# huzi96/gaussian-pcloud-render

Hardware: AMD Instinct MI355X
Metric: rendered frames/sec at 1080p (fwd+bwd), THuman-800K (higher is better)
Workload: dtype f32

## Files before the change

### gaussian-pcloud-render_amd/csrc/binning.hip

```cpp
#include "common.hpp"
#include "tile_cull.hpp"

namespace gsr {

__device__ __forceinline__ uint64_t agent_load(const uint64_t* p)
{
    return __hip_atomic_load(p, __ATOMIC_RELAXED, __HIP_MEMORY_SCOPE_AGENT);
}
__device__ __forceinline__ void agent_store(uint64_t* p, uint64_t v)
{
    __hip_atomic_store(p, v, __ATOMIC_RELAXED, __HIP_MEMORY_SCOPE_AGENT);
}

#ifdef GSR_STATS
constexpr int DUP_REC = 65536;
__device__ unsigned g_dup_rec[DUP_REC][4];
#define DUP_T(var) const unsigned long long var = wall_clock64()
#define DUP_ADD(i, v) do { if (threadIdx.x == 0) { const unsigned r_ = blockIdx.y * gridDim.x + s_ticket; if (r_ < DUP_REC) g_dup_rec[r_][i] = (unsigned)(v); } } while (0)
int debug_dup_times(unsigned long long* out8, int reset)
{
    static unsigned host[DUP_REC][4];
    if (hipMemcpyFromSymbol(host, HIP_SYMBOL(g_dup_rec), sizeof(host)) != hipSuccess) return -1;
    for (int i = 0; i < 8; i++) out8[i] = 0;
    for (int r = 0; r < DUP_REC; r++) {
// ... 272 lines not shown
    return check_launch(L, "duplicate");
}

constexpr int RANGE_SAMPLE = 4096;
constexpr int RANGE_MAX_SAMPLES = 8192;

template <typename KeyT>
__device__ __forceinline__ uint32_t lower_bound_keys(const KeyT* __restrict__ keys, uint32_t n, const uint32_t* __restrict__ samples,
                                                     uint32_t ns, uint32_t t)
{
    uint32_t lo = 0, hi = n;
    if (ns != 0) {
        uint32_t a = 0, b = ns;
        while (a < b) {
            const uint32_t m = (a + b) >> 1;
            if (samples[m] < t) a = m + 1; else b = m;
        }
        if (a == 0) return 0;
        lo = (a - 1) * RANGE_SAMPLE + 1;
        hi = a < ns ? a * RANGE_SAMPLE : n;
    }
    while (lo < hi) {
        const uint32_t m = (lo + hi) >> 1;
        if ((uint32_t)keys[m] < t) lo = m + 1; else hi = m;
    }
    return lo;
}

constexpr int RANGE_TILES_PER_WG = 255;
template <typename KeyT>
__global__ __launch_bounds__(256) void k_tile_ranges(const uint64_t* __restrict__ counters, size_t g_stride, int64_t cap,
                                                     const KeyT* __restrict__ keys, size_t b_stride, uint2* __restrict__ ranges,
                                                     size_t iv_stride, int T)
{
    __shared__ uint32_t samples[RANGE_MAX_SAMPLES];
    __shared__ uint32_t bound[256];
    const uint32_t view = blockIdx.y;
    const uint64_t n64 = at_view(counters, g_stride, view)[CNT_NUM_RENDERED];
    const uint32_t n = (uint32_t)(n64 < (uint64_t)cap ? n64 : (uint64_t)cap);
    keys = at_view(keys, b_stride, view);
    ranges = at_view(ranges, iv_stride, view);
    uint32_t ns = (n + RANGE_SAMPLE - 1) / RANGE_SAMPLE;
    if (ns > RANGE_MAX_SAMPLES) ns = 0;
    for (uint32_t j = threadIdx.x; j < ns; j += 256) samples[j] = (uint32_t)keys[(size_t)j * RANGE_SAMPLE];
    __syncthreads();
    const int t = blockIdx.x * RANGE_TILES_PER_WG + threadIdx.x;
    bound[threadIdx.x] = (t < T && n != 0) ? lower_bound_keys(keys, n, samples, ns, (uint32_t)t) : n;
    __syncthreads();
    if (threadIdx.x >= RANGE_TILES_PER_WG || t >= T) return;
    const uint32_t first = bound[threadIdx.x], last = bound[threadIdx.x + 1];
    ranges[t] = first < last ? make_uint2(first, last) : make_uint2(0u, 0u);
}

int launch_tile_ranges(const Launch& L, const Batch& B, const uint32_t* sorted_keys, int T, bool key16)
{
    const dim3 grid((unsigned)div_up(T, RANGE_TILES_PER_WG), B.V);
    if (key16)
        hipLaunchKernelGGL(k_tile_ranges<uint16_t>, grid, dim3(256), 0, L.stream, B.g.counters, B.g_stride, B.b.cap,
                           (const uint16_t*)sorted_keys, B.b_stride, B.iv.ranges, B.iv_stride, T);
    else
        hipLaunchKernelGGL(k_tile_ranges<uint32_t>, grid, dim3(256), 0, L.stream, B.g.counters, B.g_stride, B.b.cap, sorted_keys,
                           B.b_stride, B.iv.ranges, B.iv_stride, T);
    return check_launch(L, "tile_ranges");
}

constexpr int ORD_BUCKETS = 128;

__device__ __forceinline__ uint32_t work_bucket(uint32_t len)
{
    if (len == 0) return ORD_BUCKETS - 1;
    const uint32_t msb = 31u - (uint32_t)__builtin_clz(len);
    const uint32_t frac = msb >= 2 ? (len >> (msb - 2)) & 3u : 0u;
    const uint32_t rank = msb * 4u + frac;
    return (ORD_BUCKETS - 2) - (rank < ORD_BUCKETS - 2 ? rank : ORD_BUCKETS - 2);
}

__device__ __forceinline__ uint32_t work_estimate(uint32_t len, float knee, float expo)
{
    if (knee <= 0.f || (float)len <= knee) return len;
    return (uint32_t)(knee * __builtin_amdgcn_exp2f(expo * __builtin_amdgcn_logf(knee / (float)len)));
}

__global__ __launch_bounds__(1024) void k_tile_order(int T, const uint2* __restrict__ ranges, uint32_t* __restrict__ tile_order,
                                                     size_t iv_stride, float knee, float expo)
{
    ranges = at_view(ranges, iv_stride, blockIdx.x);
    tile_order = at_view(tile_order, iv_stride, blockIdx.x);
    __shared__ uint32_t cnt[ORD_BUCKETS];
    __shared__ uint32_t cur[ORD_BUCKETS];
    const uint32_t lane = threadIdx.x & 63;
    const uint64_t lt_mask = (1ull << lane) - 1ull;
    if (threadIdx.x < ORD_BUCKETS) cnt[threadIdx.x] = 0;
    __syncthreads();
    const int T_pad = (T + 1023) / 1024 * 1024;
    for (int pass = 0; pass < 2; pass++) {
        for (int t = threadIdx.x; t < T_pad; t += 1024) {
            const bool ok = t < T;
            uint32_t b = 0;
            if (ok) b = work_bucket(work_estimate(ranges[t].y - ranges[t].x, knee, expo));
            const bool empty = ok && b == ORD_BUCKETS - 1;
            const uint64_t em = __ballot(empty);
            uint32_t slot = 0;
            if (pass == 0) {
                if (empty) { if ((em & lt_mask) == 0) atomicAdd(&cnt[b], (uint32_t)__popcll(em)); }
                else if (ok) atomicAdd(&cnt[b], 1u);
            } else {
                uint32_t basev = 0;
                const int leader = em ? (int)__builtin_ctzll(em) : 0;
                if (empty && (int)lane == leader) basev = atomicAdd(&cur[b], (uint32_t)__popcll(em));
                basev = __shfl(basev, leader, 64);
                if (empty) slot = basev + (uint32_t)__popcll(em & lt_mask);
                else if (ok) slot = atomicAdd(&cur[b], 1u);
                if (ok) tile_order[slot] = (uint32_t)t;
            }
        }
        __syncthreads();
        if (pass == 0) {
            if (threadIdx.x < 64) {
                const uint32_t a0 = cnt[2 * lane], a1 = cnt[2 * lane + 1];
                uint32_t inc = a0 + a1;
#pragma unroll
                for (int d = 1; d < 64; d <<= 1) {
                    const uint32_t n = __shfl_up(inc, d, 64);
                    if (lane >= (uint32_t)d) inc += n;
                }
                cur[2 * lane] = inc - a0 - a1;
                cur[2 * lane + 1] = inc - a1;
            }
            __syncthreads();
        }
    }
}

static void order_params(float& knee, float& expo)
{
    static const float k = [] { const char* e = getenv("GSR_ORDER_KNEE"); return e ? (float)atof(e) : 2048.f; }();
    static const float x = [] { const char* e = getenv("GSR_ORDER_EXP"); return e ? (float)atof(e) : 0.3f; }();
    knee = k;
    expo = x;
}

int launch_tile_order(const Launch& L, const Batch& B, int T)
{
    float knee, expo;
    order_params(knee, expo);
    hipLaunchKernelGGL(k_tile_order, dim3(B.V), dim3(1024), 0, L.stream, T, B.iv.ranges, B.iv.tile_order, B.iv_stride, knee, expo);
    return check_launch(L, "tile_order");
}

constexpr int BWD_CLEAR_BLOCKS = 64;
__global__ __launch_bounds__(1024) void k_bwd_items(int T, int chunk_shift, const uint32_t* __restrict__ need, uint32_t* __restrict__ items,
                                                    uint32_t* __restrict__ count, size_t iv_stride, const uint64_t* __restrict__ counters,
                                                    size_t g_stride, float* __restrict__ grad_rec, size_t gr_stride, size_t gr_bytes)
{
    if (blockIdx.y != 0) {
        if (at_view(counters, g_stride, blockIdx.x)[CNT_BWD_DIRTY] == 0) return;
        zero_region(reinterpret_cast<char*>(at_view(grad_rec, gr_stride, blockIdx.x)), gr_bytes,
                    (size_t)(blockIdx.y - 1) * 1024 + threadIdx.x, (size_t)BWD_CLEAR_BLOCKS * 1024);
        return;
    }
    need = at_view(need, iv_stride, blockIdx.x);
    items = at_view(items, iv_stride, blockIdx.x);
    count = at_view(count, iv_stride, blockIdx.x);
    if (threadIdx.x < 8) count[BWD_QUEUE_WORD + threadIdx.x] = 0;
    __shared__ uint32_t cnt[ORD_BUCKETS];
    __shared__ uint32_t cur[ORD_BUCKETS];
    const uint32_t lane = threadIdx.x & 63;
    if (threadIdx.x < ORD_BUCKETS) cnt[threadIdx.x] = 0;
    __syncthreads();
    const uint32_t full_bucket = work_bucket(1u << chunk_shift);
    for (int pass = 0; pass < 2; pass++) {
        for (int t = threadIdx.x; t < T; t += 1024) {
            const uint32_t n = need[t];
            if (n == 0) continue;
            uint32_t n_full = n >> chunk_shift;
            if (n_full > BWD_MAX_CHUNKS - 1) n_full = BWD_MAX_CHUNKS - 1;
            const uint32_t rest = n - (n_full << chunk_shift);
            if (pass == 0) {
                if (n_full) atomicAdd(&cnt[full_bucket], n_full);
                if (rest) atomicAdd(&cnt[work_bucket(rest)], 1u);
            } else {
                if (n_full) {
                    const uint32_t slot = atomicAdd(&cur[full_bucket], n_full);
                    for (uint32_t c = 0; c < n_full; c++) items[slot + c] = (uint32_t)t | (c << BWD_TILE_BITS);
                }
                if (rest) items[atomicAdd(&cur[work_bucket(rest)], 1u)] = (uint32_t)t | (n_full << BWD_TILE_BITS);
            }
        }
        __syncthreads();
        if (pass == 0) {
            if (threadIdx.x < 64) {
                const uint32_t a0 = cnt[2 * lane], a1 = cnt[2 * lane + 1];
                uint32_t inc = a0 + a1;
#pragma unroll
                for (int d = 1; d < 64; d <<= 1) {
                    const uint32_t n = __shfl_up(inc, d, 64);
                    if (lane >= (uint32_t)d) inc += n;
                }
                cur[2 * lane] = inc - a0 - a1;
                cur[2 * lane + 1] = inc - a1;
                if (lane == 63) count[0] = inc;
            }
            __syncthreads();
        }
    }
}

int launch_bwd_items(const Launch& L, const Batch& B, int T, int P)
{
    hipLaunchKernelGGL(k_bwd_items, dim3(B.V, 1 + BWD_CLEAR_BLOCKS), dim3(1024), 0, L.stream, T, B.chunk_shift(), B.iv.tile_need, B.iv.bwd_items,
                       B.iv.bwd_count, B.iv_stride, B.g.counters, B.g_stride, B.grad_rec, B.gr_stride, grad_rec_bytes(P));
    return check_launch(L, "bwd_items");
}

}
```

### gaussian-pcloud-render_amd/csrc/common.hpp

```cpp
#pragma once
#include <hip/hip_runtime.h>
#include <stdint.h>

#include <type_traits>

#include "../../include/gsr.h"

#if defined(__HIP_DEVICE_COMPILE__) && !defined(__gfx950__)
#error "libgsr_hip is written for gfx950 (MI355X) only: build with --offload-arch=gfx950"
#endif

namespace gsr {

constexpr int TILE_X = 16;
constexpr int TILE_Y = 16;
constexpr int TILE_PIX = TILE_X * TILE_Y;

constexpr int RS_THREADS = 256;
constexpr int RS_WAVES = RS_THREADS / 64;
#ifndef GSR_RS_ITEMS
#define GSR_RS_ITEMS 16
#endif
constexpr int RS_ITEMS = GSR_RS_ITEMS;
constexpr int RS_TILE = RS_THREADS * RS_ITEMS;
constexpr int RADIX_BITS = 8;
constexpr int RADIX = 1 << RADIX_BITS;

constexpr int RS_ITEMS_SMALL = 8;
constexpr int RS_TILE_SMALL = RS_THREADS * RS_ITEMS_SMALL;
inline int sort_hist_stride(int64_t n, int tile = RS_TILE) { return (int)(((n + tile - 1) / tile + 15) / 16 * 16); }

constexpr int DUP_THREADS = 256;
#ifndef GSR_DUP_G
#define GSR_DUP_G 4
#endif
constexpr int DUP_G = GSR_DUP_G;
constexpr int DUP_BLOCK = DUP_THREADS * DUP_G;
#ifndef GSR_DUP_COPIES
#define GSR_DUP_COPIES 8
#endif
constexpr int DUP_COPIES = GSR_DUP_COPIES;

inline size_t align_up(size_t v, size_t a) { return (v + a - 1) / a * a; }
inline int64_t div_up(int64_t a, int64_t b) { return (a + b - 1) / b; }

template <typename T>
__host__ __device__ __forceinline__ T* at_view(T* p, size_t stride_bytes, uint32_t view)
{
    using B = typename std::conditional<std::is_const<T>::value, const char, char>::type;
    return (T*)((B*)p + stride_bytes * view);
}

struct __attribute__((aligned(64))) Splat {
    float4 q0, q1, q2, q3;
};

constexpr int GRAD_REC_WORDS = 16;
inline size_t grad_rec_bytes(int P) { return ((size_t)(P > 0 ? P : 1) * GRAD_REC_WORDS * sizeof(float) + 255) / 256 * 256; }

constexpr int CNT_NUM_RENDERED = 0;
constexpr int CNT_TRAP = 1;
constexpr int CNT_STALL = 2;
constexpr int CNT_NUM_REFERENCE = 4;
constexpr int LAND_NUM_REFERENCE = 3;
constexpr int CNT_BWD_DIRTY = 3;

struct GeomView {
    Splat* splat;
    uint32_t* tiles_touched;
    uint8_t* clamped;
    uint32_t* dkey[2];
    uint32_t* dval[2];
    uint32_t* hist;
    uint32_t* totals;
    uint32_t* blk_minmax;
    uint32_t* sortctl;
    uint64_t* dup_status;
    uint64_t* counters;
    char* zero_begin;
    size_t zero_bytes;
    size_t bytes;
};

constexpr int BWD_CHUNK_SHIFT_MIN = 9;
#ifndef GSR_CHUNK_V
#define GSR_CHUNK_V 2
#endif
__host__ __device__ inline int bwd_chunk_shift(int V) { return V >= GSR_CHUNK_V ? 10 : 9; }
constexpr int BWD_MAX_CHUNKS = 32;
constexpr int BWD_QUEUE_WORD = 8;
constexpr int BWD_TILE_BITS = 27;

struct BinView {
    uint32_t* key[2];
    uint32_t* val[2];
    uint32_t* hist;
    uint32_t* totals;
    float4* ckpt;
    int64_t cap;
    size_t bytes;
};

struct ImageView {
    uint32_t* tile_need;
    uint32_t* bwd_count;
    uint2* ranges;
    float* final_T;
    uint32_t* n_contrib;
    uint32_t* tile_order;
    float* accum;
    uint32_t* bwd_items;
    char* zero_begin;
    size_t zero_bytes;
    size_t bytes;
};

template <typename T>
inline void carve(char*& cur, T*& ptr, size_t count)
{
    ptr = reinterpret_cast<T*>(cur);
    cur += align_up(count * sizeof(T), 256);
}

inline GeomView geom_view(void* base, int P)
{
    GeomView g;
    char* cur = reinterpret_cast<char*>(base);
    const size_t p = (size_t)(P > 0 ? P : 1);
    const size_t nblk = (size_t)sort_hist_stride((int64_t)p, RS_TILE_SMALL);
    carve(cur, g.splat, p);
    carve(cur, g.tiles_touched, p);
    carve(cur, g.clamped, p);
    carve(cur, g.dkey[0], p);
    carve(cur, g.dkey[1], p);
    carve(cur, g.dval[0], p);
    carve(cur, g.dval[1], p);
    carve(cur, g.hist, RADIX * nblk);
    carve(cur, g.totals, (size_t)RADIX);
    carve(cur, g.blk_minmax, 2 * nblk);
    carve(cur, g.sortctl, (size_t)4);
    g.zero_begin = cur;
// ... 222 lines not shown
```

### gaussian-pcloud-render_amd/csrc/preprocess.hip

```cpp
#include "common.hpp"
#include "splat_math.hpp"
#include "tile_cull.hpp"

namespace gsr {

template <int deg>
__device__ __forceinline__ V3 sh_to_rgb_t(V3 pos, V3 campos, const float* sh, uint32_t* clamp_mask)
{
    V3 dir = pos - campos;
    const float len = sqrtf(dot3(dir, dir));
    dir = v3(dir.x / len, dir.y / len, dir.z / len);
#define SHV(k) v3(sh[3 * (k)], sh[3 * (k) + 1], sh[3 * (k) + 2])
    V3 result = kSH_C0 * SHV(0);
    if constexpr (deg > 0) {
        const float x = dir.x, y = dir.y, z = dir.z;
        result = ((result - (kSH_C1 * y) * SHV(1)) + (kSH_C1 * z) * SHV(2)) - (kSH_C1 * x) * SHV(3);
        if constexpr (deg > 1) {
            const float xx = x * x, yy = y * y, zz = z * z;
            const float xy = x * y, yz = y * z, xz = x * z;
            result = result + (kSH_C2[0] * xy) * SHV(4);
            result = result + (kSH_C2[1] * yz) * SHV(5);
            result = result + (kSH_C2[2] * (2.0f * zz - xx - yy)) * SHV(6);
            result = result + (kSH_C2[3] * xz) * SHV(7);
            result = result + (kSH_C2[4] * (xx - yy)) * SHV(8);
            if constexpr (deg > 2) {
                result = result + (kSH_C3[0] * y * (3.0f * xx - yy)) * SHV(9);
                result = result + (kSH_C3[1] * xy * z) * SHV(10);
                result = result + (kSH_C3[2] * y * (4.0f * zz - xx - yy)) * SHV(11);
                result = result + (kSH_C3[3] * z * (2.0f * zz - 3.0f * xx - 3.0f * yy)) * SHV(12);
                result = result + (kSH_C3[4] * x * (4.0f * zz - xx - yy)) * SHV(13);
                result = result + (kSH_C3[5] * z * (xx - yy)) * SHV(14);
                result = result + (kSH_C3[6] * x * (xx - 3.0f * yy)) * SHV(15);
            }
        }
    }
#undef SHV
    result.x += 0.5f;
    result.y += 0.5f;
    result.z += 0.5f;
    *clamp_mask = (result.x < 0 ? 1u : 0u) | (result.y < 0 ? 2u : 0u) | (result.z < 0 ? 4u : 0u);
    return v3(fmax_(result.x, 0.0f), fmax_(result.y, 0.0f), fmax_(result.z, 0.0f));
}

__device__ __forceinline__ V3 sh_to_rgb(int deg, V3 pos, V3 campos, const float* __restrict__ sh, uint32_t* clamp_mask)
{
    switch (deg) {
    case 0: return sh_to_rgb_t<0>(pos, campos, sh, clamp_mask);
    case 1: return sh_to_rgb_t<1>(pos, campos, sh, clamp_mask);
    case 2: return sh_to_rgb_t<2>(pos, campos, sh, clamp_mask);
    default: return sh_to_rgb_t<3>(pos, campos, sh, clamp_mask);
    }
}

__device__ __forceinline__ float ndc_to_pix(float v, int S) { return (float)((((double)v + 1.0) * (double)S - 1.0) * 0.5); }

__device__ __forceinline__ uint32_t clamp_tile(float f, uint32_t grid)
{
    int v = (int)f;
    v = v > 0 ? v : 0;
    return grid < (uint32_t)v ? grid : (uint32_t)v;
}

struct PreArgs {
    int P, D, M, W, H, V, vpt;
    float tanfovx, tanfovy, focal_x, focal_y, scale_modifier;
    int prefiltered, need_backward, reference_lists;
    uint32_t gridx, gridy;
    const float *means3D, *shs, *colors_precomp, *opacities, *scales, *rotations, *cov3D_precomp;
    const float *view, *proj, *campos;
    Splat* splat;
    uint32_t* tiles_touched;
    uint8_t* clamped;
    uint32_t* dkey;
    float* grad_rec;
    uint64_t* counters;
    char* g_zero;
    size_t g_zero_bytes, g_stride, gr_stride;
    char* iv_zero;
    size_t iv_zero_bytes, iv_stride;
    int* radii;
};

template <int DEG>
__global__ __launch_bounds__(256) void k_preprocess(PreArgs a)
{
    const int v_first = blockIdx.y * a.vpt, v_last = v_first + a.vpt < a.V ? v_first + a.vpt : a.V;
    const int idx_raw = blockIdx.x * 256 + threadIdx.x;
    {
        const size_t gtid = (size_t)blockIdx.x * 256 + threadIdx.x, nthr = (size_t)gridDim.x * 256;
        for (int vw = v_first; vw < v_last; vw++) {
            if (gtid == 0) {
                at_view(a.counters, a.g_stride, vw)[CNT_STALL] = 0;
                at_view(a.counters, a.g_stride, vw)[CNT_BWD_DIRTY] = 0;
            }
            zero_region(a.g_zero + a.g_stride * vw, a.g_zero_bytes, gtid, nthr);
            zero_region(a.iv_zero + a.iv_stride * vw, a.iv_zero_bytes, gtid, nthr);
        }
    }
    const bool valid = idx_raw < a.P;
    const int idx = valid ? idx_raw : a.P - 1;
    __shared__ float4 xpose[4][256];

    const V3 p_orig = v3(a.means3D[3 * idx], a.means3D[3 * idx + 1], a.means3D[3 * idx + 2]);
    float cov6[6];
    if (a.cov3D_precomp) {
#pragma unroll
        for (int i = 0; i < 6; i++) cov6[i] = a.cov3D_precomp[6 * (size_t)idx + i];
    } else {
        const V3 sc = v3(a.scales[3 * idx], a.scales[3 * idx + 1], a.scales[3 * idx + 2]);
        const float4 q = *reinterpret_cast<const float4*>(a.rotations + 4 * (size_t)idx);
        cov3d_from_scale_rot(sc, a.scale_modifier, q, cov6, nullptr);
    }
    const float opacity = a.opacities[idx];
    V3 rgb_pre = v3(0, 0, 0);
    constexpr int NSH = 3 * (DEG + 1) * (DEG + 1);
    float shv[NSH];
    if (a.colors_precomp) {
        rgb_pre = v3(a.colors_precomp[3 * idx], a.colors_precomp[3 * idx + 1], a.colors_precomp[3 * idx + 2]);
    } else {
        const float* shp = a.shs + (size_t)idx * a.M * 3;
#pragma unroll
        for (int i = 0; i < NSH; i++) shv[i] = shp[i];
    }

    for (int vw = v_first; vw < v_last; vw++) {
        float view[16], proj[16];
#pragma unroll
        for (int i = 0; i < 16; i++) {
            view[i] = a.view[16 * vw + i];
            proj[i] = a.proj[16 * vw + i];
        }

        int radius_out = 0;
        uint32_t tiles = 0, etiles = 0, key = 0xFFFFFFFFu, cmask = 0;
        uint2 rect = make_uint2(0, 0), spans = make_uint2(0, 0);
        bool spans_valid = false;
        Splat s;
        s.q0 = make_float4(0, 0, 0, 0);
        s.q1 = make_float4(0, 0, 0, 0);
        s.q2 = make_float4(0, 0, 0, 0);

        const V3 p_view = xform_point_4x3(p_orig, view);
        if (p_view.z <= 0.2f) {
            if (a.prefiltered && valid) at_view(a.counters, a.g_stride, vw)[CNT_TRAP] = 1;
        } else {
            const float hx = ((proj[0] * p_orig.x + proj[4] * p_orig.y) + proj[8] * p_orig.z) + proj[12];
            const float hy = ((proj[1] * p_orig.x + proj[5] * p_orig.y) + proj[9] * p_orig.z) + proj[13];
            const float hw = ((proj[3] * p_orig.x + proj[7] * p_orig.y) + proj[11] * p_orig.z) + proj[15];
            const float p_w = 1.0f / (hw + 0.0000001f);
            const float proj_x = hx * p_w, proj_y = hy * p_w;

            const Cov2D c = cov2d_project(p_orig, a.focal_x, a.focal_y, a.tanfovx, a.tanfovy, cov6, view);
            const float cov_x = c.cov.m[0][0] + 0.3f;
            const float cov_y = c.cov.m[0][1];
            const float cov_z = c.cov.m[1][1] + 0.3f;

            const float det = (cov_x * cov_z - cov_y * cov_y);
            if (det != 0.0f) {
                const float det_inv = 1.f / det;
                const float conic_x = cov_z * det_inv, conic_y = -cov_y * det_inv, conic_z = cov_x * det_inv;

                const float mid = 0.5f * (cov_x + cov_z);
                const float lambda1 = mid + sqrtf(fmax_(0.1f, mid * mid - det));
                const float lambda2 = mid - sqrtf(fmax_(0.1f, mid * mid - det));
                const float my_radius = ceilf(3.f * sqrtf(fmax_(lambda1, lambda2)));
                const float px = ndc_to_pix(proj_x, a.W), py = ndc_to_pix(proj_y, a.H);

                const float r = (float)(int)my_radius;
                const uint32_t minx = clamp_tile((px - r) / (float)TILE_X, a.gridx);
                const uint32_t miny = clamp_tile((py - r) / (float)TILE_Y, a.gridy);
                const uint32_t maxx = clamp_tile((((px + r) + (float)TILE_X) - 1.0f) / (float)TILE_X, a.gridx);
                const uint32_t maxy = clamp_tile((((py + r) + (float)TILE_Y) - 1.0f) / (float)TILE_Y, a.gridy);
                const uint32_t ntiles = (maxx - minx) * (maxy - miny);
                if (ntiles != 0) {
                    V3 rgb = rgb_pre;
                    if (!a.colors_precomp) {
                        const V3 cam = v3(a.campos[3 * vw], a.campos[3 * vw + 1], a.campos[3 * vw + 2]);
                        rgb = sh_to_rgb_t<DEG>(p_orig, cam, shv, &cmask);
                    }
                    radius_out = (int)my_radius;
                    tiles = ntiles;
                    key = __float_as_uint(p_view.z);
                    rect = make_uint2(minx | (miny << 16), maxx | (maxy << 16));
                    etiles = a.reference_lists ? ntiles
                                               : clip_rect_to_footprint(px, py, cov_x, cov_y, cov_z, det, conic_x, conic_y, conic_z,
#ifdef GSR_NO_SPANS
                                                                        opacity, r, rect, a.gridx, a.gridy);
#else
                                                                        opacity, r, rect, a.gridx, a.gridy, &spans, &spans_valid);
#endif
                    s.q0 = make_float4(px, py, conic_x, conic_y);
                    s.q1 = make_float4(conic_z, opacity, rgb.x, rgb.y);
                    s.q2 = make_float4(rgb.z, p_view.z, 0.f, 0.f);
                }
            }
        }

        if (valid) {
            a.radii[(size_t)vw * a.P + idx] = radius_out;
            at_view(a.tiles_touched, a.g_stride, vw)[idx] = tiles;
            at_view(a.dkey, a.g_stride, vw)[idx] = key;
        }
        const float4 q3 = spans_valid ? make_float4(__uint_as_float(rect.x), __uint_as_float(spans.x), __uint_as_float(spans.y),
                                                    __uint_as_float(tiles | SPANS_FLAG))
                                      : make_float4(__uint_as_float(rect.x), __uint_as_float(rect.y), __uint_as_float(etiles),
                                                    __uint_as_float(tiles));
        const int wave_first = idx_raw - (int)(threadIdx.x & 63);
        const bool full_wave = wave_first + 64 <= a.P;
        if (full_wave) {
            float4* mine = xpose[threadIdx.x >> 6] + 4 * (threadIdx.x & 63);
            mine[0] = s.q0; mine[1] = s.q1; mine[2] = s.q2; mine[3] = q3;
            __builtin_amdgcn_wave_barrier();
            const float4* rd = xpose[threadIdx.x >> 6] + (threadIdx.x & 63);
            float4* out = reinterpret_cast<float4*>(at_view(a.splat, a.g_stride, vw) + wave_first) + (threadIdx.x & 63);
            const float4 t0 = rd[0], t1 = rd[64], t2 = rd[128], t3 = rd[192];
            out[0] = t0; out[64] = t1; out[128] = t2; out[192] = t3;
            __builtin_amdgcn_wave_barrier();
        } else if (valid) {
            Splat* sp = at_view(a.splat, a.g_stride, vw) + idx;
            sp->q0 = s.q0;
            sp->q1 = s.q1;
            sp->q2 = s.q2;
            sp->q3 = q3;
        }
        if (a.need_backward && valid) {
            at_view(a.clamped, a.g_stride, vw)[idx] = (uint8_t)cmask;
            const float4 z = make_float4(0.f, 0.f, 0.f, 0.f);
            if (full_wave) {
                float4* recw = reinterpret_cast<float4*>(at_view(a.grad_rec, a.gr_stride, vw) + (size_t)wave_first * GRAD_REC_WORDS) + (threadIdx.x & 63);
                recw[0] = z; recw[64] = z; recw[128] = z; recw[192] = z;
            } else {
                float4* rec = reinterpret_cast<float4*>(at_view(a.grad_rec, a.gr_stride, vw) + (size_t)idx * GRAD_REC_WORDS);
                rec[0] = z; rec[1] = z; rec[2] = z; rec[3] = z;
            }
        }
    }
}

int launch_preprocess(const Launch& L, const gsr_params& p, const Batch& B, int* radii)
{
    const GeomView& g = B.g;
    PreArgs a;
    a.P = p.P; a.D = p.D; a.M = p.M; a.W = p.W; a.H = p.H;
    a.tanfovx = p.tanfovx; a.tanfovy = p.tanfovy;
    a.focal_y = p.H / (2.0f * p.tanfovy);
    a.focal_x = p.W / (2.0f * p.tanfovx);
    a.scale_modifier = p.scale_modifier;
    a.prefiltered = p.prefiltered;
    a.need_backward = p.need_backward;
    a.reference_lists = p.reference_lists;
    a.gridx = (uint32_t)((p.W + TILE_X - 1) / TILE_X);
    a.gridy = (uint32_t)((p.H + TILE_Y - 1) / TILE_Y);
    a.means3D = p.means3D; a.shs = p.shs; a.colors_precomp = p.colors_precomp; a.opacities = p.opacities;
    a.scales = p.scales; a.rotations = p.rotations; a.cov3D_precomp = p.cov3D_precomp;
    a.view = p.viewmatrix; a.proj = p.projmatrix; a.campos = p.campos;
    a.splat = g.splat; a.tiles_touched = g.tiles_touched; a.clamped = g.clamped;
    a.dkey = g.dkey[0]; a.radii = radii; a.counters = g.counters; a.grad_rec = B.grad_rec; a.gr_stride = B.gr_stride;
    a.g_zero = g.zero_begin; a.g_zero_bytes = g.zero_bytes; a.g_stride = B.g_stride;
    a.iv_zero = B.iv.zero_begin; a.iv_zero_bytes = B.iv.zero_bytes; a.iv_stride = B.iv_stride;
    const int blocks = (p.P + 255) / 256;
    a.V = B.V;
    a.vpt = 1;
    while (a.vpt < B.V && (int64_t)blocks * div_up(B.V, a.vpt * 2) >= 2048) a.vpt *= 2;
    if (a.vpt > B.V) a.vpt = B.V;
    const dim3 grid(blocks, (unsigned)div_up(B.V, a.vpt));
    switch (p.shs ? p.D : 0) {
    case 0: hipLaunchKernelGGL(k_preprocess<0>, grid, dim3(256), 0, L.stream, a); break;
    case 1: hipLaunchKernelGGL(k_preprocess<1>, grid, dim3(256), 0, L.stream, a); break;
    case 2: hipLaunchKernelGGL(k_preprocess<2>, grid, dim3(256), 0, L.stream, a); break;
    default: hipLaunchKernelGGL(k_preprocess<3>, grid, dim3(256), 0, L.stream, a); break;
    }
    return check_launch(L, "preprocess");
}

__global__ __launch_bounds__(256) void k_recolor(int P, int D, int M, const float* __restrict__ means3D,
                                                 const float* __restrict__ shs, const float* __restrict__ colors_precomp,
                                                 const float* __restrict__ campos, const uint32_t* __restrict__ tiles_touched,
                                                 Splat* __restrict__ splat, uint8_t* __restrict__ clamped, size_t g_stride,
                                                 size_t colors_view_stride)
{
    const uint32_t vw = blockIdx.y;
    if (colors_precomp) colors_precomp += colors_view_stride * vw;
    tiles_touched = at_view(tiles_touched, g_stride, vw);
    splat = at_view(splat, g_stride, vw);
    if (campos) campos += 3 * vw;
    const int idx = blockIdx.x * 256 + threadIdx.x;
    if (idx >= P || tiles_touched[idx] == 0) return;
    V3 rgb;
    uint32_t cmask = 0;
    if (colors_precomp) {
        rgb = v3(colors_precomp[3 * idx], colors_precomp[3 * idx + 1], colors_precomp[3 * idx + 2]);
    } else {
        const V3 pos = v3(means3D[3 * idx], means3D[3 * idx + 1], means3D[3 * idx + 2]);
        rgb = sh_to_rgb(D, pos, v3(campos[0], campos[1], campos[2]), shs + (size_t)idx * M * 3, &cmask);
    }
    float* rec = reinterpret_cast<float*>(splat + idx);
    rec[6] = rgb.x;
    rec[7] = rgb.y;
    rec[8] = rgb.z;
    if (clamped) at_view(clamped, g_stride, vw)[idx] = (uint8_t)cmask;
}

int launch_recolor(const Launch& L, const gsr_params& p, const Batch& B, size_t colors_view_stride)
{
    hipLaunchKernelGGL(k_recolor, dim3((p.P + 255) / 256, B.V), dim3(256), 0, L.stream, p.P, p.D, p.M, p.means3D, p.shs,
                       p.colors_precomp, p.campos, B.g.tiles_touched, B.g.splat, p.need_backward ? B.g.clamped : nullptr, B.g_stride,
                       colors_view_stride);
    return check_launch(L, "recolor");
}

__global__ __launch_bounds__(256) void k_mark_visible(int P, const float* __restrict__ means3D,
                                                      const float* __restrict__ view, uint8_t* __restrict__ present)
{
    const int idx = blockIdx.x * 256 + threadIdx.x;
    if (idx >= P) return;
    const V3 p = v3(means3D[3 * idx], means3D[3 * idx + 1], means3D[3 * idx + 2]);
    const float z = ((view[2] * p.x + view[6] * p.y) + view[10] * p.z) + view[14];
    present[idx] = !(z <= 0.2f);
}

int launch_mark_visible(const Launch& L, int P, const float* means3D, const float* view, uint8_t* present)
{
    hipLaunchKernelGGL(k_mark_visible, dim3((P + 255) / 256), dim3(256), 0, L.stream, P, means3D, view, present);
    return check_launch(L, "mark_visible");
}

}
```

### gaussian-pcloud-render_amd/csrc/render_fwd.hip

```cpp
#include <atomic>
#include <cstdlib>

#include "common.hpp"
#include "tile_cull.hpp"

namespace gsr {


struct RenderArgs {
    const uint2* ranges;
    const uint32_t* tile_order;
    const uint32_t* point_list;
    const Splat* splat;
    int W, H, gridx, num_tiles, chunk_shift;
    const float* bg;
    float* out_color;
    float* final_T;
    uint32_t* n_contrib;
    uint32_t* tile_need;
    float4* ckpt;
    float* accum;
    uint32_t V;
    size_t g_stride, b_stride, iv_stride;
    const float* extra;
    size_t extra_vstride;
    size_t extra_hi_vstride;
    const float* extra_hi;
    const float* extra_scale;
    const float* bg_extra;
    float* out_extra;
    float4* xckpt;
    float* xaccum;
    size_t x_stride;
};

typedef float f32x4 __attribute__((ext_vector_type(4)));

__device__ __forceinline__ void prefetch16(f32x4& dst, const void* p)
{
    asm volatile("global_load_dwordx4 %0, %1, off" : "=v"(dst) : "v"(p) : "memory");
}
__device__ __forceinline__ void prefetch4(uint32_t& dst, const void* p)
{
    asm volatile("global_load_dword %0, %1, off" : "=v"(dst) : "v"(p) : "memory");
}
__device__ __forceinline__ void prefetch4f(float& dst, const void* p)
{
    asm volatile("global_load_dword %0, %1, off" : "=v"(dst) : "v"(p) : "memory");
}
__device__ __forceinline__ void retire_prefetch(f32x4& a, f32x4& b, float& c, uint32_t& d)
{
    asm volatile("s_waitcnt vmcnt(0)" : "+v"(a), "+v"(b), "+v"(c), "+v"(d)::"memory");
}

__device__ __forceinline__ void retire_prefetch_x(f32x4& a, f32x4& b, float& c, uint32_t& d, f32x4& e, f32x4& f)
{
    asm volatile("s_waitcnt vmcnt(0)" : "+v"(a), "+v"(b), "+v"(c), "+v"(d), "+v"(e), "+v"(f)::"memory");
}

__device__ __forceinline__ float exp_nonpos(float x)
{
    const float ph = x * 0x1.715476p+0f;
    float pl = __builtin_fmaf(x, 0x1.715476p+0f, -ph);
    pl = __builtin_fmaf(x, 0x1.4ae0bep-26f, pl);
    const float e = __builtin_rintf(ph);
    const float r = __builtin_amdgcn_exp2f((ph - e) + pl);
    return __builtin_ldexpf(r, (int)e);
}

typedef float f32x2 __attribute__((ext_vector_type(2)));

__device__ __forceinline__ f32x2 exp_nonpos2(f32x2 x)
{
    const f32x2 c = {0x1.715476p+0f, 0x1.715476p+0f}, cc = {0x1.4ae0bep-26f, 0x1.4ae0bep-26f};
    const f32x2 ph = x * c;
    f32x2 pl = __builtin_elementwise_fma(x, c, -ph);
    pl = __builtin_elementwise_fma(x, cc, pl);
    const f32x2 e = {__builtin_rintf(ph.x), __builtin_rintf(ph.y)};
    const f32x2 a = (ph - e) + pl;
    f32x2 r;
    r.x = __builtin_ldexpf(__builtin_amdgcn_exp2f(a.x), (int)e.x);
    r.y = __builtin_ldexpf(__builtin_amdgcn_exp2f(a.y), (int)e.y);
    return r;
}

constexpr int PAIR_WORDS = 20;
template <int NX>
struct PairRec {
    f32x4 xy;
    f32x4 ab;
    f32x4 co;
    f32x4 rg;
    f32x2 b;
    uint2 pos;
    f32x4 ex[NX > 0 ? NX / 2 : 1];
};
template <int NX>
__device__ __forceinline__ PairRec<NX> read_pair(const float* lds, int pair)
{
    const float* p = lds + pair * (PAIR_WORDS + 2 * NX);
    PairRec<NX> r;
    r.xy = *(const f32x4*)(p + 0);
    r.ab = *(const f32x4*)(p + 4);
    r.co = *(const f32x4*)(p + 8);
    r.rg = *(const f32x4*)(p + 12);
    r.b = *(const f32x2*)(p + 16);
    r.pos = *(const uint2*)(p + 18);
#pragma unroll
    for (int j = 0; j < NX / 2; j++) r.ex[j] = *(const f32x4*)(p + PAIR_WORDS + 4 * j);
    return r;
}

__device__ __forceinline__ bool stage_entry(float* stage, int pw, uint32_t slot, uint32_t nsurv, const f32x4& c0, const f32x4& c1, float c2b,
                                            uint32_t my_pos)
{
    float* p = stage + (slot >> 1) * pw + (slot & 1u);
    p[0] = c0.x; p[2] = c0.y; p[4] = c0.z; p[6] = c0.w; p[8] = c1.x; p[10] = c1.y;
    float* pc = stage + (slot >> 1) * pw + 12 + 2 * (slot & 1u);
    pc[0] = c1.z; pc[1] = c1.w;
    p[16] = c2b;
    uint32_t* pp = (uint32_t*)p;
    pp[18] = my_pos;
    const bool lone = slot + 1 == nsurv && (slot & 1u) == 0;
    if (lone) {
        p[1] = c0.x; p[3] = c0.y; p[5] = c0.z; p[7] = c0.w; p[9] = c1.x; p[11] = 0.f;
        pc[2] = c1.z; pc[3] = c1.w;
        p[17] = c2b;
        pp[19] = my_pos;
    }
    return lone;
}

#ifdef GSR_STATS
constexpr int FW_REC = 1 << 19;
__device__ unsigned g_fwd_rec[FW_REC][8];
__device__ unsigned g_fwd_hw[FW_REC][2];
int debug_fwd_records(unsigned* out, int n)
{
    static unsigned host[FW_REC][8], hw[FW_REC][2];
    if (hipMemcpyFromSymbol(host, HIP_SYMBOL(g_fwd_rec), sizeof(host)) != hipSuccess) return -1;
    if (hipMemcpyFromSymbol(hw, HIP_SYMBOL(g_fwd_hw), sizeof(hw)) != hipSuccess) return -1;
    if (n > FW_REC) n = FW_REC;
    for (int r = 0; r < n; r++) {
        for (int i = 0; i < 8; i++) out[r * 10 + i] = host[r][i];
        out[r * 10 + 8] = hw[r][0]; out[r * 10 + 9] = hw[r][1];
    }
    return n;
}
#define FW_T(var) const unsigned long long var = wall_clock64()
int debug_fwd_times(unsigned long long* out8, int reset)
{
    static unsigned host[FW_REC][8];
    if (hipMemcpyFromSymbol(host, HIP_SYMBOL(g_fwd_rec), sizeof(host)) != hipSuccess) return -1;
    for (int i = 0; i < 8; i++) out8[i] = 0;
    for (int r = 0; r < FW_REC; r++) {
        for (int i = 0; i < 7; i++) out8[i] += host[r][i];
        if (host[r][0] > out8[7]) out8[7] = host[r][0];
    }
    if (reset) {
        for (int r = 0; r < FW_REC; r++) for (int i = 0; i < 8; i++) host[r][i] = 0;
        if (hipMemcpyToSymbol(HIP_SYMBOL(g_fwd_rec), host, sizeof(host)) != hipSuccess) return -1;
    }
    return 0;
}
#endif

template <int NX>
__global__ __launch_bounds__(64) void k_render_forward(RenderArgs a)
{
#ifdef GSR_STATS
    FW_T(tw0);
    unsigned long long tw_wait = 0, tw_stage = 0, tw_eval = 0, n_rounds = 0, n_pairs = 0;
    unsigned live_cnt = 64, n_pairs_le8 = 0, n_pairs_le16 = 0, n_pairs_le32 = 0;
#endif
    static_assert(NX == 0 || NX == 4 || NX == 8, "extra channels come in quads");
    constexpr int PW = PAIR_WORDS + 2 * NX;
    const uint32_t group = blockIdx.x >> 5;
    const uint32_t view = group % a.V;
    const uint32_t order_slot = (group / a.V) * 8u + (blockIdx.x & 7u);
    if (order_slot >= (uint32_t)a.num_tiles) return;
    a.ranges = at_view(a.ranges, a.iv_stride, view);
    a.tile_order = at_view(a.tile_order, a.iv_stride, view);
    a.final_T = at_view(a.final_T, a.iv_stride, view);
    a.n_contrib = at_view(a.n_contrib, a.iv_stride, view);
    a.tile_need = at_view(a.tile_need, a.iv_stride, view);
    a.accum = at_view(a.accum, a.iv_stride, view);
    a.point_list = at_view(a.point_list, a.b_stride, view);
    if (a.ckpt) a.ckpt = at_view(a.ckpt, a.b_stride, view);
    a.splat = at_view(a.splat, a.g_stride, view);
    a.out_color += (size_t)view * 3u * (size_t)a.W * (size_t)a.H;
    if (NX > 0) a.extra += (size_t)view * a.extra_vstride;
    float4* const xckpt = NX > 0 && a.xckpt != nullptr ? at_view(a.xckpt, a.x_stride, view) : nullptr;
    const bool x_split = NX > 4 && a.extra_hi != nullptr;
    const float* const x_hi = x_split ? a.extra_hi + (size_t)view * a.extra_hi_vstride : a.extra + 4;
    const uint32_t x_nx = x_split ? 4u : (uint32_t)NX;
    const uint32_t tile = a.tile_order[order_slot];
    const uint32_t q = (blockIdx.x >> 3) & 3u;
    const uint32_t lane = threadIdx.x;
    const uint32_t tx = tile % (uint32_t)a.gridx, ty = tile / (uint32_t)a.gridx;
    const uint32_t x0 = tx * TILE_X + (q & 1u) * 8u, y0 = ty * TILE_Y + (q >> 1) * 8u;
    const uint32_t px = x0 + (lane & 7u), py = y0 + (lane >> 3);
    const bool inside = px < (uint32_t)a.W && py < (uint32_t)a.H;
    const float pixf_x = (float)px, pixf_y = (float)py;
    const float x0f = (float)x0, y0f = (float)y0;
    float bx0 = x0f, by0 = y0f, bx1 = x0f + 7.f, by1 = y0f + 7.f;

    __shared__ __attribute__((aligned(16))) float stage[33 * PW];

    const uint2 range = a.ranges[tile];
    const int total = (int)(range.y - range.x);

    float T = 1.0f;
    f32x2 C01 = {0.f, 0.f};
    float C2 = 0.f;
    f32x2 CX[NX > 0 ? NX / 2 : 1];
#pragma unroll
    for (int j = 0; j < (NX > 0 ? NX / 2 : 1); j++) CX[j] = f32x2{0.f, 0.f};
    f32x4 xs0 = {1.f, 1.f, 1.f, 1.f}, xs1 = {1.f, 1.f, 1.f, 1.f};
    if (NX > 0 && a.extra_scale != nullptr) {
        const float* sc = a.extra_scale + (size_t)view * NX;
        xs0 = f32x4{sc[0], sc[1], sc[2], sc[3]};
        if (NX > 4) xs1 = f32x4{sc[4], sc[5], sc[6], sc[7]};
    }
    uint32_t last_contributor = 0;
    uint32_t stop_at = 0;
    bool crossed = false;
    bool done = !inside;
    bool all_done = __all(done);
#ifdef GSR_STATS
    live_cnt = (unsigned)__popcll(__ballot(!done));
#endif
    if (!all_done) {
        int ax, ay, bx, by;
        live_box(__ballot(!done), ax, ay, bx, by);
        bx0 = x0f + (float)ax; by0 = y0f + (float)ay; bx1 = x0f + (float)bx; by1 = y0f + (float)by;
    }

    if (!all_done && total > 0) {
        const uint32_t* plist = a.point_list + range.x;
        const int last = total - 1;
        f32x4 c0, c1, n0, n1;
        f32x4 cx0 = {0.f, 0.f, 0.f, 0.f}, cx1 = cx0, nx0 = cx0, nx1 = cx0;
        float c2b, n2b;
        uint32_t id_cur, id_nxt, id_nn;
        {
            prefetch4(id_cur, plist + ((int)lane < total ? (int)lane : last));
            prefetch4(id_nxt, plist + (64 + (int)lane < total ? 64 + (int)lane : last));
            asm volatile("s_waitcnt vmcnt(0)" : "+v"(id_cur), "+v"(id_nxt)::"memory");
            const Splat* sp = a.splat + id_cur;
            prefetch16(c0, &sp->q0);
            prefetch16(c1, &sp->q1);
            prefetch4f(c2b, &sp->q2);
            if (NX > 0) {
                prefetch16(cx0, a.extra + (size_t)id_cur * x_nx);
                if (NX > 4) prefetch16(cx1, x_hi + (size_t)id_cur * x_nx);
                retire_prefetch_x(c0, c1, c2b, id_nxt, cx0, cx1);
            } else {
                retire_prefetch(c0, c1, c2b, id_nxt);
            }
        }
        for (int base = 0; base < total; base += 64) {
            {
                const Splat* sp = a.splat + id_nxt;
                prefetch16(n0, &sp->q0);
                prefetch16(n1, &sp->q1);
                prefetch4f(n2b, &sp->q2);
                if (NX > 0) {
                    prefetch16(nx0, a.extra + (size_t)id_nxt * x_nx);
                    if (NX > 4) prefetch16(nx1, x_hi + (size_t)id_nxt * x_nx);
                }
                const int i2 = base + 128 + (int)lane;
                prefetch4(id_nn, plist + (i2 < total ? i2 : last));
            }

            if (a.ckpt != nullptr && base != 0 && (base & ((1 << a.chunk_shift) - 1)) == 0 && (base >> a.chunk_shift) < BWD_MAX_CHUNKS) {
                const size_t slot = (size_t)(range.x >> a.chunk_shift) + (size_t)(base >> a.chunk_shift);
                a.ckpt[slot * 256 + q * 64 + lane] = make_float4(T, C01.x, C01.y, C2);
                if (NX > 0 && xckpt != nullptr) {
#pragma unroll
                    for (int j = 0; j < NX / 4; j++)
                        xckpt[(slot * (NX / 4) + j) * 256 + q * 64 + lane] = make_float4(CX[2 * j].x, CX[2 * j].y, CX[2 * j + 1].x, CX[2 * j + 1].y);
// ... 135 lines not shown
        unsigned* r_ = g_fwd_rec[blockIdx.x];
        r_[0] = (unsigned)(tw1 - tw0); r_[1] = (unsigned)tw_wait; r_[2] = (unsigned)tw_stage; r_[3] = (unsigned)tw_eval;
        r_[4] = 1u; r_[5] = (unsigned)n_rounds; r_[6] = (unsigned)n_pairs;
        r_[7] = n_pairs_le8 | (n_pairs_le16 << 10) | (n_pairs_le32 << 20);
        g_fwd_hw[blockIdx.x][0] = __builtin_amdgcn_s_getreg(63492) | (__builtin_amdgcn_s_getreg(63508) << 28);
        g_fwd_hw[blockIdx.x][1] = (unsigned)tw0;
    }
#endif
    {
        uint32_t need = inside ? (done ? stop_at : (uint32_t)total) : 0u;
#pragma unroll
        for (int d = 32; d >= 1; d >>= 1) {
            const uint32_t o = __shfl_xor(need, d, 64);
            need = need > o ? need : o;
        }
        if (lane == 0 && need != 0) atomicMax(&a.tile_need[tile], need);
    }

    if (inside) {
        const size_t pix = (size_t)py * a.W + px, N = (size_t)a.W * a.H;
        a.final_T[pix] = T;
        a.n_contrib[pix] = last_contributor;
        a.out_color[pix] = C01.x + T * a.bg[0];
        a.out_color[N + pix] = C01.y + T * a.bg[1];
        a.out_color[2 * N + pix] = C2 + T * a.bg[2];
        if (NX > 0) {
            float* ox = a.out_extra + (size_t)view * NX * N + pix;
#pragma unroll
            for (int j = 0; j < NX / 2; j++) {
                ox[(size_t)(2 * j) * N] = CX[j].x + T * a.bg_extra[2 * j];
                ox[(size_t)(2 * j + 1) * N] = CX[j].y + T * a.bg_extra[2 * j + 1];
            }
        }
        if (crossed) {
            a.accum[pix] = C01.x;
            a.accum[N + pix] = C01.y;
            a.accum[2 * N + pix] = C2;
            if (NX > 0 && xckpt != nullptr) {
                float* xa = at_view(a.xaccum, a.x_stride, view) + pix;
#pragma unroll
                for (int j = 0; j < NX / 2; j++) {
                    xa[(size_t)(2 * j) * N] = CX[j].x;
                    xa[(size_t)(2 * j + 1) * N] = CX[j].y;
                }
            }
        }
    }
}

__device__ __forceinline__ void swap_halves2(float& a_lo, float& a_hi, float& b_lo, float& b_hi)
{
    const auto a = __builtin_amdgcn_permlane32_swap(__float_as_uint(a_lo), __float_as_uint(a_hi), false, false);
    const auto b = __builtin_amdgcn_permlane32_swap(__float_as_uint(b_lo), __float_as_uint(b_hi), false, false);
    a_lo = __uint_as_float(a[0]);
    a_hi = __uint_as_float(a[1]);
    b_lo = __uint_as_float(b[0]);
    b_hi = __uint_as_float(b[1]);
}

__global__ __launch_bounds__(64) void k_render_forward_half(RenderArgs a)
{
#ifdef GSR_STATS
    FW_T(tw0);
    unsigned long long tw_wait = 0, tw_stage = 0, tw_eval = 0, n_rounds = 0, n_pairs = 0;
#endif
    constexpr int PW = PAIR_WORDS;
    const uint32_t group = blockIdx.x >> 6;
    const uint32_t view = group % a.V;
    const uint32_t order_slot = (group / a.V) * 8u + (blockIdx.x & 7u);
    if (order_slot >= (uint32_t)a.num_tiles) return;
    a.ranges = at_view(a.ranges, a.iv_stride, view);
    a.tile_order = at_view(a.tile_order, a.iv_stride, view);
    a.final_T = at_view(a.final_T, a.iv_stride, view);
    a.n_contrib = at_view(a.n_contrib, a.iv_stride, view);
    a.tile_need = at_view(a.tile_need, a.iv_stride, view);
    a.accum = at_view(a.accum, a.iv_stride, view);
    a.point_list = at_view(a.point_list, a.b_stride, view);
    if (a.ckpt) a.ckpt = at_view(a.ckpt, a.b_stride, view);
    a.splat = at_view(a.splat, a.g_stride, view);
    a.out_color += (size_t)view * 3u * (size_t)a.W * (size_t)a.H;
    const uint32_t tile = a.tile_order[order_slot];
    const uint32_t sb = (blockIdx.x >> 3) & 7u, q = sb >> 1, hf = sb & 1u;
    const uint32_t lane = threadIdx.x, pl = lane & 31u, eg = lane >> 5;
    const uint32_t tx = tile % (uint32_t)a.gridx, ty = tile / (uint32_t)a.gridx;
    const uint32_t x0 = tx * TILE_X + (q & 1u) * 8u, y0 = ty * TILE_Y + (q >> 1) * 8u + hf * 4u;
    const uint32_t px = x0 + (pl & 7u), py = y0 + (pl >> 3);
    const bool inside = px < (uint32_t)a.W && py < (uint32_t)a.H;
    const float pixf_x = (float)px, pixf_y = (float)py;
    const float x0f = (float)x0, y0f = (float)y0;
    float bx0 = x0f, by0 = y0f, bx1 = x0f + 7.f, by1 = y0f + 3.f;

    __shared__ __attribute__((aligned(16))) float stage[35 * PW];

    const uint2 range = a.ranges[tile];
    const int total = (int)(range.y - range.x);

    float T = 1.0f;
    f32x2 C01 = {0.f, 0.f};
    float C2 = 0.f;
    uint32_t last_contributor = 0;
    uint32_t stop_at = 0;
    bool crossed = false;
    bool done = !inside;
    bool all_done = __all(done);
    if (!all_done) {
        int ax, ay, bx, by;
        live_box(__ballot(!done) & 0xFFFFFFFFull, ax, ay, bx, by);
        bx0 = x0f + (float)ax; by0 = y0f + (float)ay; bx1 = x0f + (float)bx; by1 = y0f + (float)by;
    }

    if (!all_done && total > 0) {
        const uint32_t* plist = a.point_list + range.x;
        const int last = total - 1;
        f32x4 c0, c1, n0, n1;
        float c2b, n2b;
        uint32_t id_cur, id_nxt, id_nn;
        {
            prefetch4(id_cur, plist + ((int)lane < total ? (int)lane : last));
            prefetch4(id_nxt, plist + (64 + (int)lane < total ? 64 + (int)lane : last));
            asm volatile("s_waitcnt vmcnt(0)" : "+v"(id_cur), "+v"(id_nxt)::"memory");
            const Splat* sp = a.splat + id_cur;
            prefetch16(c0, &sp->q0);
            prefetch16(c1, &sp->q1);
            prefetch4f(c2b, &sp->q2);
            retire_prefetch(c0, c1, c2b, id_nxt);
        }
        for (int base = 0; base < total; base += 64) {
            {
                const Splat* sp = a.splat + id_nxt;
                prefetch16(n0, &sp->q0);
                prefetch16(n1, &sp->q1);
                prefetch4f(n2b, &sp->q2);
                const int i2 = base + 128 + (int)lane;
                prefetch4(id_nn, plist + (i2 < total ? i2 : last));
            }
            if (a.ckpt != nullptr && base != 0 && (base & ((1 << a.chunk_shift) - 1)) == 0 && (base >> a.chunk_shift) < BWD_MAX_CHUNKS) {
                const size_t slot = (size_t)(range.x >> a.chunk_shift) + (size_t)(base >> a.chunk_shift);
                if (eg == 0) a.ckpt[slot * 256 + q * 64 + hf * 32u + pl] = make_float4(T, C01.x, C01.y, C2);
                crossed = true;
            }
#ifdef GSR_STATS
            FW_T(ts0);
            n_rounds++;
#endif
            const bool valid = base + (int)lane < total;
            const bool touch = valid && may_touch_rect(c0.x, c0.y, c0.z, c0.w, c1.x, c1.y, bx0, by0, bx1, by1);
            const uint64_t mask = __ballot(touch);
            if (mask != 0) {
                const uint32_t slot = __builtin_amdgcn_mbcnt_hi((uint32_t)(mask >> 32), __builtin_amdgcn_mbcnt_lo((uint32_t)mask, 0u));
                const uint32_t nsurv = (uint32_t)__popcll(mask);
                const int npairs = (int)((nsurv + 1u) >> 1);
                if (touch) stage_entry(stage, PW, slot, nsurv, c0, c1, c2b, (uint32_t)(base + (int)lane + 1));
                if ((npairs & 1) && lane < (uint32_t)PW) stage[npairs * PW + lane] = 0.f;
                const int nsteps = (npairs + 1) >> 1;
                struct StepRec {
                    f32x4 xy, ab, co, rgA, rgB;
                    f32x2 bA, bB;
                    uint2 posA, posB;
                };
                auto load_step = [&](int st) {
                    StepRec r;
                    const float* po = stage + (2 * st + (int)eg) * PW;
                    const float* pa = stage + (2 * st) * PW;
                    r.xy = *(const f32x4*)(po + 0);
                    r.ab = *(const f32x4*)(po + 4);
                    r.co = *(const f32x4*)(po + 8);
// ... 89 lines not shown
#ifdef GSR_STATS
            { FW_T(ts4); tw_wait += ts4 - ts3; }
#endif
            if (all_done) break;
            c0 = n0; c1 = n1; c2b = n2b;
            id_cur = id_nxt;
            id_nxt = id_nn;
        }
    }
#ifdef GSR_STATS
    if (lane == 0 && blockIdx.x < (unsigned)FW_REC) {
        FW_T(tw1);
        unsigned* r_ = g_fwd_rec[blockIdx.x];
        r_[0] = (unsigned)(tw1 - tw0); r_[1] = (unsigned)tw_wait; r_[2] = (unsigned)tw_stage; r_[3] = (unsigned)tw_eval;
        r_[4] = 1u; r_[5] = (unsigned)n_rounds; r_[6] = (unsigned)n_pairs; r_[7] = (unsigned)total;
        g_fwd_hw[blockIdx.x][0] = __builtin_amdgcn_s_getreg(63492) | (__builtin_amdgcn_s_getreg(63508) << 28);
        g_fwd_hw[blockIdx.x][1] = (unsigned)tw0;
    }
#endif
    {
        uint32_t need = inside ? (done ? stop_at : (uint32_t)total) : 0u;
#pragma unroll
        for (int d = 32; d >= 1; d >>= 1) {
            const uint32_t o = __shfl_xor(need, d, 64);
            need = need > o ? need : o;
        }
        if (lane == 0 && need != 0) atomicMax(&a.tile_need[tile], need);
    }
    if (inside && eg == 0) {
        const size_t pix = (size_t)py * a.W + px, N = (size_t)a.W * a.H;
        a.final_T[pix] = T;
        a.n_contrib[pix] = last_contributor;
        a.out_color[pix] = C01.x + T * a.bg[0];
        a.out_color[N + pix] = C01.y + T * a.bg[1];
        a.out_color[2 * N + pix] = C2 + T * a.bg[2];
        if (crossed) {
            a.accum[pix] = C01.x;
            a.accum[N + pix] = C01.y;
            a.accum[2 * N + pix] = C2;
        }
    }
}

static std::atomic<int> g_fwd_half_v{-1};
int forward_half_views(int set)
{
    if (set >= 0) g_fwd_half_v.store(set);
    int v = g_fwd_half_v.load();
    if (v < 0) {
        const char* e = getenv("GSR_FWD_HALF_V");
        v = e ? atoi(e) : 1;
        if (v < 0) v = 0;
        g_fwd_half_v.store(v);
    }
    return v;
}

int launch_render_forward(const Launch& L, const gsr_params& p, const Batch& B, const uint32_t* point_list, float* out_color,
                          bool with_ckpt, const ExtraChannels* X)
{
    RenderArgs a;
    a.ranges = B.iv.ranges;
    a.tile_order = B.iv.tile_order;
    a.point_list = point_list;
    a.splat = B.g.splat;
    a.W = p.W; a.H = p.H;
    a.gridx = (p.W + TILE_X - 1) / TILE_X;
    const int gridy = (p.H + TILE_Y - 1) / TILE_Y;
    a.bg = p.bg;
    a.out_color = out_color;
    a.final_T = B.iv.final_T;
    a.n_contrib = B.iv.n_contrib;
    a.tile_need = B.iv.tile_need;
    a.ckpt = with_ckpt ? B.b.ckpt : nullptr;
    a.accum = B.iv.accum;
    a.V = (uint32_t)B.V;
    a.g_stride = B.g_stride; a.b_stride = B.b_stride; a.iv_stride = B.iv_stride;
    const int T = a.gridx * gridy;
    a.num_tiles = T;
    a.chunk_shift = B.chunk_shift();
    a.extra = nullptr; a.extra_scale = nullptr; a.bg_extra = nullptr; a.out_extra = nullptr; a.extra_vstride = 0;
    a.extra_hi = nullptr; a.extra_hi_vstride = 0;
    a.xckpt = nullptr; a.xaccum = nullptr; a.x_stride = 0;
    const dim3 grid((unsigned)div_up(T, 8) * 32u * (unsigned)B.V);
    if (X != nullptr && X->nx > 0) {
        a.extra = X->values; a.extra_scale = X->view_scale; a.bg_extra = X->bg; a.out_extra = X->out; a.extra_vstride = X->view_stride;
        a.extra_hi = X->values_hi; a.extra_hi_vstride = X->hi_view_stride;
        if (with_ckpt && X->state.ckpt != nullptr) {
            a.xckpt = X->state.ckpt; a.xaccum = X->state.accum; a.x_stride = X->state_stride;
        }
        if (X->nx == 4) hipLaunchKernelGGL(k_render_forward<4>, grid, dim3(64), 0, L.stream, a);
        else hipLaunchKernelGGL(k_render_forward<8>, grid, dim3(64), 0, L.stream, a);
    } else if (B.V <= forward_half_views(-1)) {
        hipLaunchKernelGGL(k_render_forward_half, dim3((unsigned)div_up(T, 8) * 64u * (unsigned)B.V), dim3(64), 0, L.stream, a);
    } else {
        hipLaunchKernelGGL(k_render_forward<0>, grid, dim3(64), 0, L.stream, a);
    }
    return check_launch(L, "render_forward");
}

}
```

Measured before the change: 2138.

## Move grad record zeroing from preprocess into forward render blocks

Removes the per-Gaussian zeroing of backward gradient records from the preprocess kernel. The forward render kernels now clear the whole grad_rec buffer in chunks, split across live tile blocks, with chunk sizes computed by the tile-order kernel and stored in bookkeeping words. The aim is to hide the clearing traffic inside the latency-bound render blocks instead of making preprocess do it. The cost is extra stores at the start of every render block, more work for heavy tiles, and a reliance on bwd_count words 1 and 2 not being overwritten before the render kernel reads them.

New measurement: 2149 (median of 6 runs). No clear change (+0.5%).

```diff
diff --git a/gaussian-pcloud-render_amd/csrc/binning.hip b/gaussian-pcloud-render_amd/csrc/binning.hip
--- a/gaussian-pcloud-render_amd/csrc/binning.hip
+++ b/gaussian-pcloud-render_amd/csrc/binning.hip
@@ -378,10 +378,12 @@
 }
 
 __global__ __launch_bounds__(1024) void k_tile_order(int T, const uint2* __restrict__ ranges, uint32_t* __restrict__ tile_order,
-                                                     size_t iv_stride, float knee, float expo)
+                                                     uint32_t* __restrict__ bookkeeping, size_t iv_stride, size_t gr_bytes, float knee,
+                                                     float expo)
 {
     ranges = at_view(ranges, iv_stride, blockIdx.x);
     tile_order = at_view(tile_order, iv_stride, blockIdx.x);
+    bookkeeping = at_view(bookkeeping, iv_stride, blockIdx.x);
     __shared__ uint32_t cnt[ORD_BUCKETS];
     __shared__ uint32_t cur[ORD_BUCKETS];
     const uint32_t lane = threadIdx.x & 63;
@@ -422,6 +424,11 @@
                 }
                 cur[2 * lane] = inc - a0 - a1;
                 cur[2 * lane + 1] = inc - a1;
+                if (lane == 63) {
+                    const uint32_t n_live = inc - a1;
+                    bookkeeping[CLEAR_LIVE_WORD] = n_live;
+                    bookkeeping[CLEAR_KB_WORD] = clear_chunk_kb(gr_bytes, clear_tiles(n_live, (uint32_t)T));
+                }
             }
             __syncthreads();
         }
@@ -440,7 +447,8 @@
 {
     float knee, expo;
     order_params(knee, expo);
-    hipLaunchKernelGGL(k_tile_order, dim3(B.V), dim3(1024), 0, L.stream, T, B.iv.ranges, B.iv.tile_order, B.iv_stride, knee, expo);
+    hipLaunchKernelGGL(k_tile_order, dim3(B.V), dim3(1024), 0, L.stream, T, B.iv.ranges, B.iv.tile_order, B.iv.bwd_count, B.iv_stride,
+                       B.gr_stride, knee, expo);
     return check_launch(L, "tile_order");
 }
 
diff --git a/gaussian-pcloud-render_amd/csrc/common.hpp b/gaussian-pcloud-render_amd/csrc/common.hpp
--- a/gaussian-pcloud-render_amd/csrc/common.hpp
+++ b/gaussian-pcloud-render_amd/csrc/common.hpp
@@ -57,6 +57,19 @@
 
 constexpr int GRAD_REC_WORDS = 16;
 inline size_t grad_rec_bytes(int P) { return ((size_t)(P > 0 ? P : 1) * GRAD_REC_WORDS * sizeof(float) + 255) / 256 * 256; }
+constexpr int CLEAR_LIVE_WORD = 1;
+constexpr int CLEAR_KB_WORD = 2;
+constexpr int CLEAR_MIN_TILES = 64;
+__host__ __device__ inline uint32_t clear_tiles(uint32_t n_live, uint32_t T)
+{
+    const uint32_t floor_ = T < (uint32_t)CLEAR_MIN_TILES ? T : (uint32_t)CLEAR_MIN_TILES;
+    return n_live > floor_ ? n_live : floor_;
+}
+__host__ __device__ inline uint32_t clear_chunk_kb(size_t gr_bytes, uint32_t n_clear)
+{
+    const uint32_t kb = (uint32_t)((gr_bytes + 1023) >> 10), chunks = 4u * (n_clear ? n_clear : 1u);
+    return (kb + chunks - 1) / chunks;
+}
 
 constexpr int CNT_NUM_RENDERED = 0;
 constexpr int CNT_TRAP = 1;
diff --git a/gaussian-pcloud-render_amd/csrc/preprocess.hip b/gaussian-pcloud-render_amd/csrc/preprocess.hip
--- a/gaussian-pcloud-render_amd/csrc/preprocess.hip
+++ b/gaussian-pcloud-render_amd/csrc/preprocess.hip
@@ -72,10 +72,9 @@
     uint32_t* tiles_touched;
     uint8_t* clamped;
     uint32_t* dkey;
-    float* grad_rec;
     uint64_t* counters;
     char* g_zero;
-    size_t g_zero_bytes, g_stride, gr_stride;
+    size_t g_zero_bytes, g_stride;
     char* iv_zero;
     size_t iv_zero_bytes, iv_stride;
     int* radii;
@@ -223,17 +222,7 @@
             sp->q2 = s.q2;
             sp->q3 = q3;
         }
-        if (a.need_backward && valid) {
-            at_view(a.clamped, a.g_stride, vw)[idx] = (uint8_t)cmask;
-            const float4 z = make_float4(0.f, 0.f, 0.f, 0.f);
-            if (full_wave) {
-                float4* recw = reinterpret_cast<float4*>(at_view(a.grad_rec, a.gr_stride, vw) + (size_t)wave_first * GRAD_REC_WORDS) + (threadIdx.x & 63);
-                recw[0] = z; recw[64] = z; recw[128] = z; recw[192] = z;
-            } else {
-                float4* rec = reinterpret_cast<float4*>(at_view(a.grad_rec, a.gr_stride, vw) + (size_t)idx * GRAD_REC_WORDS);
-                rec[0] = z; rec[1] = z; rec[2] = z; rec[3] = z;
-            }
-        }
+        if (a.need_backward && valid) at_view(a.clamped, a.g_stride, vw)[idx] = (uint8_t)cmask;
     }
 }
 
@@ -255,7 +244,7 @@
     a.scales = p.scales; a.rotations = p.rotations; a.cov3D_precomp = p.cov3D_precomp;
     a.view = p.viewmatrix; a.proj = p.projmatrix; a.campos = p.campos;
     a.splat = g.splat; a.tiles_touched = g.tiles_touched; a.clamped = g.clamped;
-    a.dkey = g.dkey[0]; a.radii = radii; a.counters = g.counters; a.grad_rec = B.grad_rec; a.gr_stride = B.gr_stride;
+    a.dkey = g.dkey[0]; a.radii = radii; a.counters = g.counters;
     a.g_zero = g.zero_begin; a.g_zero_bytes = g.zero_bytes; a.g_stride = B.g_stride;
     a.iv_zero = B.iv.zero_begin; a.iv_zero_bytes = B.iv.zero_bytes; a.iv_stride = B.iv_stride;
     const int blocks = (p.P + 255) / 256;
diff --git a/gaussian-pcloud-render_amd/csrc/render_fwd.hip b/gaussian-pcloud-render_amd/csrc/render_fwd.hip
--- a/gaussian-pcloud-render_amd/csrc/render_fwd.hip
+++ b/gaussian-pcloud-render_amd/csrc/render_fwd.hip
@@ -32,7 +32,24 @@
     float4* xckpt;
     float* xaccum;
     size_t x_stride;
+    float* grad_rec;
+    size_t gr_stride, gr_bytes;
+    const uint32_t* clear_info;
 };
+
+__device__ __forceinline__ void clear_grad_records(const RenderArgs& a, uint32_t view, uint32_t order_slot, uint32_t q, uint32_t part,
+                                                   uint32_t nparts, uint32_t lane)
+{
+    const uint32_t* info = at_view(a.clear_info, a.iv_stride, view);
+    const uint32_t n_live = info[CLEAR_LIVE_WORD], chunk_kb = info[CLEAR_KB_WORD];
+    if (order_slot >= clear_tiles(n_live, (uint32_t)a.num_tiles)) return;
+    const size_t chunk_bytes = (size_t)chunk_kb << 10;
+    const size_t begin = (size_t)(order_slot * 4u + q) * chunk_bytes;
+    const size_t end = begin + chunk_bytes < a.gr_bytes ? begin + chunk_bytes : a.gr_bytes;
+    char* rec = reinterpret_cast<char*>(at_view(a.grad_rec, a.gr_stride, view));
+    for (size_t off = begin + ((size_t)part << 10) + (size_t)lane * 16u; off < end; off += (size_t)nparts << 10)
+        *reinterpret_cast<uint4*>(rec + off) = make_uint4(0u, 0u, 0u, 0u);
+}
 
 typedef float f32x4 __attribute__((ext_vector_type(4)));
 
@@ -197,6 +214,7 @@
     const uint32_t tile = a.tile_order[order_slot];
     const uint32_t q = (blockIdx.x >> 3) & 3u;
     const uint32_t lane = threadIdx.x;
+    if (a.grad_rec != nullptr) clear_grad_records(a, view, order_slot, q, 0u, 1u, lane);
     const uint32_t tx = tile % (uint32_t)a.gridx, ty = tile / (uint32_t)a.gridx;
     const uint32_t x0 = tx * TILE_X + (q & 1u) * 8u, y0 = ty * TILE_Y + (q >> 1) * 8u;
     const uint32_t px = x0 + (lane & 7u), py = y0 + (lane >> 3);
@@ -498,6 +516,7 @@
     const uint32_t tile = a.tile_order[order_slot];
     const uint32_t sb = (blockIdx.x >> 3) & 7u, q = sb >> 1, hf = sb & 1u;
     const uint32_t lane = threadIdx.x, pl = lane & 31u, eg = lane >> 5;
+    if (a.grad_rec != nullptr) clear_grad_records(a, view, order_slot, q, hf, 2u, lane);
     const uint32_t tx = tile % (uint32_t)a.gridx, ty = tile / (uint32_t)a.gridx;
     const uint32_t x0 = tx * TILE_X + (q & 1u) * 8u, y0 = ty * TILE_Y + (q >> 1) * 8u + hf * 4u;
     const uint32_t px = x0 + (pl & 7u), py = y0 + (pl >> 3);
@@ -753,6 +772,9 @@
     a.extra = nullptr; a.extra_scale = nullptr; a.bg_extra = nullptr; a.out_extra = nullptr; a.extra_vstride = 0;
     a.extra_hi = nullptr; a.extra_hi_vstride = 0;
     a.xckpt = nullptr; a.xaccum = nullptr; a.x_stride = 0;
+    a.grad_rec = with_ckpt ? B.grad_rec : nullptr;
+    a.gr_stride = B.gr_stride; a.gr_bytes = B.gr_stride;
+    a.clear_info = B.iv.bwd_count;
     const dim3 grid((unsigned)div_up(T, 8) * 32u * (unsigned)B.V);
     if (X != nullptr && X->nx > 0) {
         a.extra = X->values; a.extra_scale = X->view_scale; a.bg_extra = X->bg; a.out_extra = X->out; a.extra_vstride = X->view_stride;
```
